# ViktorLiang/GW-Depth

Hardware: AMD Instinct MI355X
Metric: images/sec (train fwd+bwd) 480x640 bs=8/GPU (higher is better)
Workload: dtype bf16; 1 GPU; GW-Depth full model (res50 + DETR 6+6 + 4-scale ReferTransformer + decoder) fwd+17 losses+bwd+clip+AdamW, 480x640, bs=8/GPU, dropout 0.1; global_batch=8, parallelism=dp1, launch=hipgraph, graph_segments=1, grad_buckets=8

## Files before the change

### gw_depth_amd/csrc/refattn.hip

```cpp
#include "common.h"

namespace {

struct QOp {
    const void *p;
    long ws, ts, hs;
};
struct QOpW {
    void *p;
    long ws, ts, hs;
};

template <typename T, int HD>
__device__ __forceinline__ void load_row(float (&v)[HD], const T *p) {
    if constexpr (sizeof(T) == 2) {
#pragma unroll
        for (int c = 0; c < HD; c += 8) {
            const bf16x8 x = *(const bf16x8 *)(p + c);
#pragma unroll
            for (int j = 0; j < 8; ++j) v[c + j] = (float)x[j];
        }
    } else {
#pragma unroll
        for (int c = 0; c < HD; c += 4) {
            const float4 x = *(const float4 *)(p + c);
            v[c] = x.x, v[c + 1] = x.y, v[c + 2] = x.z, v[c + 3] = x.w;
        }
    }
}

template <typename T, int HD>
__global__ void ref_scores_fwd_kernel(QOp q, const T *__restrict__ refk, T *__restrict__ ra, int B, int nwin, int R, int H, float scale) {
    const long total = (long)B * nwin * 49 * H;
    const int C = H * HD, Tn = nwin * 49;
    for (long i = (long)blockIdx.x * blockDim.x + threadIdx.x; i < total; i += (long)gridDim.x * blockDim.x) {
        const int h = (int)(i % H);
        const long bt = i / H;
        const int t = (int)(bt % Tn), b = (int)(bt / Tn);
        float qv[HD];
        load_row<T, HD>(qv, (const T *)q.p + ((long)b * nwin + t / 49) * q.ws + (long)(t % 49) * q.ts + (long)h * q.hs);
        const T *kp = refk + (long)b * R * C + h * HD;
        T *dst = ra + bt * R * H + h;
        for (int r = 0; r < R; ++r) {
            float kv[HD];
            load_row<T, HD>(kv, kp + (long)r * C);
            float acc = 0.f;
#pragma unroll
            for (int d = 0; d < HD; ++d) acc += qv[d] * kv[d];
            dst[(long)r * H] = from_f32<T>(acc * scale);
        }
    }
}

template <typename T, int HD>
__global__ void ref_scores_dq_kernel(const T *__restrict__ refk, const T *__restrict__ g, QOpW dq, int B, int nwin, int R, int H, float scale) {
    const long total = (long)B * nwin * 49 * H;
    const int C = H * HD, Tn = nwin * 49;
    for (long i = (long)blockIdx.x * blockDim.x + threadIdx.x; i < total; i += (long)gridDim.x * blockDim.x) {
        const int h = (int)(i % H);
        const long bt = i / H;
        const int t = (int)(bt % Tn), b = (int)(bt / Tn);
        const T *gp = g + bt * R * H + h;
        const T *kp = refk + (long)b * R * C + h * HD;
        float acc[HD];
#pragma unroll
        for (int d = 0; d < HD; ++d) acc[d] = 0.f;
        for (int r = 0; r < R; ++r) {
            float kv[HD];
            load_row<T, HD>(kv, kp + (long)r * C);
            const float gv = to_f32(gp[(long)r * H]);
#pragma unroll
            for (int d = 0; d < HD; ++d) acc[d] += gv * kv[d];
        }
        T *dst = (T *)dq.p + ((long)b * nwin + t / 49) * dq.ws + (long)(t % 49) * dq.ts + (long)h * dq.hs;
#pragma unroll
        for (int d = 0; d < HD; ++d) dst[d] = from_f32<T>(acc[d] * scale);
    }
}

template <typename T, int HD>
__global__ void token_reduce_kernel(const T *__restrict__ a, QOp x, float *__restrict__ out, int B, int nwin, int R, int H, float scale) {
    const int lane = threadIdx.x & 63;
    const long wave = ((long)blockIdx.x * blockDim.x + threadIdx.x) >> 6, total = (long)B * R * H;
    if (wave >= total) return;
    const int h = (int)(wave % H), r = (int)((wave / H) % R), b = (int)(wave / ((long)H * R));
    const int Tn = nwin * 49;
    const T *ap = a + ((long)b * Tn * R + r) * H + h;
    float acc[HD];
#pragma unroll
    for (int d = 0; d < HD; ++d) acc[d] = 0.f;
    for (int t = lane; t < Tn; t += 64) {
        float xv[HD];
        load_row<T, HD>(xv, (const T *)x.p + ((long)b * nwin + t / 49) * x.ws + (long)(t % 49) * x.ts + (long)h * x.hs);
        const float av = to_f32(ap[(long)t * R * H]);
#pragma unroll
        for (int d = 0; d < HD; ++d) acc[d] += av * xv[d];
    }
    float *dst = out + ((long)b * R + r) * H * HD + h * HD;
#pragma unroll
    for (int d = 0; d < HD; ++d) {
        const float s = wave_sum(acc[d]);
        if (lane == (d & 63)) dst[d] = s * scale;
    }
}

template <typename T>
__global__ void ref_mix_fwd_kernel(const T *__restrict__ ra, const T *__restrict__ refv, T *__restrict__ qnew, T *__restrict__ att_out,
                                   int R, int H, int hd, int Tn) {
    extern __shared__ float sm[];
    const long bt = blockIdx.x;
    const int C = H * hd, RH = R * H;
    const T *src = ra + bt * RH;
    for (int e = threadIdx.x; e < RH; e += blockDim.x) sm[e] = to_f32(src[e]);
    __syncthreads();
    {
        float *red = sm + RH;
        const int parts = blockDim.x / H, hh = threadIdx.x % H, pp = threadIdx.x / H;
        float m = -INFINITY;
        if (pp < parts)
            for (int r = pp; r < R; r += parts) m = fmaxf(m, sm[r * H + hh]);
        if (pp < parts) red[pp * H + hh] = m;
        __syncthreads();
        for (int q = 0; q < parts; ++q) m = fmaxf(m, red[q * H + hh]);
        __syncthreads();
        float l = 0.f;
        if (pp < parts)
            for (int r = pp; r < R; r += parts) {
                const float p = __expf(sm[r * H + hh] - m);
                sm[r * H + hh] = p;
                l += p;
            }
        if (pp < parts) red[pp * H + hh] = l;
        __syncthreads();
        l = 0.f;
        for (int q = 0; q < parts; ++q) l += red[q * H + hh];
        const float inv = 1.0f / l;
        if (pp < parts)
            for (int r = pp; r < R; r += parts) sm[r * H + hh] *= inv;
    }
    __syncthreads();
    if (att_out)
        for (int e = threadIdx.x; e < RH; e += blockDim.x) att_out[bt * RH + e] = from_f32<T>(sm[e]);
    const T *vb = refv + (bt / Tn) * R * C;
    for (int e = threadIdx.x; e < C; e += blockDim.x) {
        const int h = e / hd;
        float acc = 0.f;
        for (int r = 0; r < R; ++r) acc += sm[r * H + h] * to_f32(vb[(long)r * C + e]);
        qnew[bt * C + e] = from_f32<T>(acc);
    }
}

template <typename T>
__global__ void ref_mix_bwd_kernel(const T *__restrict__ att, const T *__restrict__ refv, const T *__restrict__ g, T *__restrict__ dra,
                                   int R, int H, int hd, int Tn) {
    extern __shared__ float sm[];
    const long bt = blockIdx.x;
    const int C = H * hd, RH = R * H;
    const int GP = hd + 1;
    float *gs = sm, *da = sm + H * GP, *dot = da + RH;
    for (int e = threadIdx.x; e < C; e += blockDim.x) gs[(e / hd) * GP + e % hd] = to_f32(g[bt * C + e]);
    __syncthreads();
    const T *vb = refv + (bt / Tn) * R * C;
    constexpr int VE = 16 / (int)sizeof(T);
    const bool vec = (hd % VE) == 0 && ((uintptr_t)vb % 16) == 0;
    for (int e = threadIdx.x; e < RH; e += blockDim.x) {
        const int r = e / H, h = e % H;
        const T *vp = vb + (long)r * C + h * hd;
        float acc = 0.f;
        if (vec) {
            for (int d = 0; d < hd; d += VE) {
                const uint4 raw = *(const uint4 *)(vp + d);
                const T *pv = (const T *)&raw;
#pragma unroll
                for (int k = 0; k < VE; ++k) acc += gs[h * GP + d + k] * to_f32(pv[k]);
            }
        } else {
            for (int d = 0; d < hd; ++d) acc += gs[h * GP + d] * to_f32(vp[d]);
        }
        da[e] = acc;
    }
    __syncthreads();
    float *part = dot + H;
    const int parts = blockDim.x / H, hh = threadIdx.x % H, pp = threadIdx.x / H;
    float av[4];
    float s = 0.f;
    int n = 0;
    if (pp < parts)
        for (int r = pp; r < R; r += parts, ++n) {
            const float a = to_f32(att[bt * RH + r * H + hh]);
            if (n < 4) av[n] = a;
            s += a * da[r * H + hh];
        }
    if (pp < parts) part[pp * H + hh] = s;
    __syncthreads();
    if (threadIdx.x < H) {
        float t = 0.f;
        for (int q = 0; q < parts; ++q) t += part[q * H + threadIdx.x];
        dot[threadIdx.x] = t;
    }
    __syncthreads();
    n = 0;
    if (pp < parts)
        for (int r = pp; r < R; r += parts, ++n) {
            const float a = n < 4 ? av[n] : to_f32(att[bt * RH + r * H + hh]);
            dra[bt * RH + r * H + hh] = from_f32<T>(a * (da[r * H + hh] - dot[hh]));
        }
}

bool shape_ok(int B, int nwin, int R, int H, int hd) { return B > 0 && nwin > 0 && R > 0 && R <= 128 && H > 0 && H <= 64 && hd > 0 && hd <= 64; }
int blocks_for(long n, int per, int cap) {
    long b = (n + per - 1) / per;
    return (int)(b > cap ? cap : (b < 1 ? 1 : b));
}

}

#define HD_SWITCH(hd, CALL)            \
    switch (hd) {                      \
        case 8: { CALL(8) } break;     \
        case 16: { CALL(16) } break;   \
        case 32: { CALL(32) } break;   \
        case 64: { CALL(64) } break;   \
        default: return -4;            \
    }

bool q_aligned(const gwd_strided *q, int32_t dtype) {
    const int a = dtype == GWD_BF16 ? 8 : 4;
    return (uintptr_t)q->p % 16 == 0 && q->ws % a == 0 && q->ts % a == 0 && q->hs % a == 0;
}

extern "C" int gwd_ref_scores_forward(const gwd_strided *q, const void *ref_k, void *ra, int32_t B, int32_t nwin, int32_t R, int32_t H,
                                      int32_t hd, float scale, int32_t dtype, void *stream) {
    if (!q || !q->p || !ref_k || !ra || !shape_ok(B, nwin, R, H, hd)) return -1;
    if (!q_aligned(q, dtype) || (uintptr_t)ref_k % 16) return -5;
    const QOp qo{q->p, q->ws, q->ts, q->hs};
    const int grid = blocks_for((long)B * nwin * 49 * H, 64, 16384);
    hipStream_t s = (hipStream_t)stream;
    if (dtype == GWD_BF16) {
#define CALL(HD_) ref_scores_fwd_kernel<__bf16, HD_><<<grid, 64, 0, s>>>(qo, (const __bf16 *)ref_k, (__bf16 *)ra, B, nwin, R, H, scale);
        HD_SWITCH(hd, CALL)
#undef CALL
    } else if (dtype == GWD_F32) {
#define CALL(HD_) ref_scores_fwd_kernel<float, HD_><<<grid, 64, 0, s>>>(qo, (const float *)ref_k, (float *)ra, B, nwin, R, H, scale);
        HD_SWITCH(hd, CALL)
#undef CALL
    } else return -2;
    GWD_CHECK_LAUNCH();
    return 0;
}

extern "C" int gwd_ref_scores_backward(const gwd_strided *q, const void *ref_k, const void *g, const gwd_strided *dq, float *d_ref_k,
                                       int32_t B, int32_t nwin, int32_t R, int32_t H, int32_t hd, float scale, int32_t dtype,
                                       void *stream) {
    if (!q || !q->p || !dq || !dq->p || !ref_k || !g || !d_ref_k || !shape_ok(B, nwin, R, H, hd)) return -1;
    if (!q_aligned(q, dtype) || (uintptr_t)ref_k % 16) return -5;
    const QOp qo{q->p, q->ws, q->ts, q->hs};
    const QOpW dqo{dq->p, dq->ws, dq->ts, dq->hs};
    const int grid = blocks_for((long)B * nwin * 49 * H, 64, 16384);
    const unsigned rgrid = (unsigned)(((long)B * R * H + 3) / 4);
    hipStream_t s = (hipStream_t)stream;
    if (dtype == GWD_BF16) {
#define CALL(HD_)                                                                                                             \
    ref_scores_dq_kernel<__bf16, HD_><<<grid, 64, 0, s>>>((const __bf16 *)ref_k, (const __bf16 *)g, dqo, B, nwin, R, H, scale);    \
    token_reduce_kernel<__bf16, HD_><<<rgrid, 256, 0, s>>>((const __bf16 *)g, qo, d_ref_k, B, nwin, R, H, scale);
        HD_SWITCH(hd, CALL)
#undef CALL
    } else if (dtype == GWD_F32) {
#define CALL(HD_)                                                                                                             \
    ref_scores_dq_kernel<float, HD_><<<grid, 64, 0, s>>>((const float *)ref_k, (const float *)g, dqo, B, nwin, R, H, scale);       \
    token_reduce_kernel<float, HD_><<<rgrid, 256, 0, s>>>((const float *)g, qo, d_ref_k, B, nwin, R, H, scale);
        HD_SWITCH(hd, CALL)
#undef CALL
    } else return -2;
    GWD_CHECK_LAUNCH();
    return 0;
}

extern "C" int gwd_ref_mix_forward(const void *ra, const void *ref_v, void *q_new, void *att, int32_t B, int32_t T, int32_t R, int32_t H,
                                   int32_t hd, int32_t dtype, void *stream) {
    if (!ra || !ref_v || !q_new || T <= 0 || !shape_ok(B, 1, R, H, hd)) return -1;
    const unsigned grid = (unsigned)((long)B * T);
    hipStream_t s = (hipStream_t)stream;
    const size_t lds = ((size_t)R * H + (size_t)(256 / H) * H) * sizeof(float);
    if (dtype == GWD_BF16) ref_mix_fwd_kernel<__bf16><<<grid, 256, lds, s>>>((const __bf16 *)ra, (const __bf16 *)ref_v, (__bf16 *)q_new, (__bf16 *)att, R, H, hd, T);
    else if (dtype == GWD_F32) ref_mix_fwd_kernel<float><<<grid, 256, lds, s>>>((const float *)ra, (const float *)ref_v, (float *)q_new, (float *)att, R, H, hd, T);
    else return -2;
    GWD_CHECK_LAUNCH();
    return 0;
}

extern "C" int gwd_ref_mix_backward(const void *att, const void *ref_v, const void *g, void *d_ra, float *d_ref_v, int32_t B, int32_t T,
                                    int32_t R, int32_t H, int32_t hd, int32_t dtype, void *stream) {
    if (!att || !ref_v || !g || !d_ra || !d_ref_v || T <= 0 || T % 49 || !shape_ok(B, 1, R, H, hd)) return -1;
    if ((uintptr_t)g % 16) return -5;
    hipStream_t s = (hipStream_t)stream;
    const size_t lds = ((size_t)H * (hd + 1) + (size_t)R * H + H + (size_t)(256 / H) * H) * sizeof(float);
    const unsigned rgrid = (unsigned)(((long)B * R * H + 3) / 4);
    const long C = (long)H * hd;
    const QOp go{g, 49 * C, C, hd};
    if (dtype == GWD_BF16) {
        ref_mix_bwd_kernel<__bf16><<<(unsigned)((long)B * T), 256, lds, s>>>((const __bf16 *)att, (const __bf16 *)ref_v, (const __bf16 *)g, (__bf16 *)d_ra, R, H, hd, T);
#define CALL(HD_) token_reduce_kernel<__bf16, HD_><<<rgrid, 256, 0, s>>>((const __bf16 *)att, go, d_ref_v, B, T / 49, R, H, 1.0f);
        HD_SWITCH(hd, CALL)
#undef CALL
    } else if (dtype == GWD_F32) {
        ref_mix_bwd_kernel<float><<<(unsigned)((long)B * T), 256, lds, s>>>((const float *)att, (const float *)ref_v, (const float *)g, (float *)d_ra, R, H, hd, T);
#define CALL(HD_) token_reduce_kernel<float, HD_><<<rgrid, 256, 0, s>>>((const float *)att, go, d_ref_v, B, T / 49, R, H, 1.0f);
        HD_SWITCH(hd, CALL)
#undef CALL
    } else return -2;
    GWD_CHECK_LAUNCH();
    return 0;
}
```

Baseline: 262.2 images/s.

## Add MFMA-based token-tiled kernels for reference attention forward and backward

Adds new bf16 kernels for hd 16/32 that tile 32 tokens per block in LDS and compute the scores, the softmax-mix and their backward passes with MFMA instructions instead of scalar per-token loops. The backward launches also fold the separate token-reduction kernel into the same grid as extra blocks that do the reductions with MFMA over transposed LDS tiles. This is meant to cut launch count, scalar FMA work and redundant global reads of the reference K/V. The cost is more complex indexing, larger LDS use per block and fallback paths when alignment checks fail.

New measurement: 264.7 images/s (median of 6 runs). About the same (+1.0%).

```diff
diff --git a/gw_depth_amd/csrc/refattn.hip b/gw_depth_amd/csrc/refattn.hip
--- a/gw_depth_amd/csrc/refattn.hip
+++ b/gw_depth_amd/csrc/refattn.hip
@@ -207,6 +207,427 @@
         }
 }
 
+namespace mf {
+
+constexpr int NTHR = 512, NWV = NTHR / 64;
+constexpr int PAD = 8;
+constexpr int LDS_TOKEN_BUDGET = 61440;
+constexpr int KT = 32, PT = KT + 8;
+constexpr int SUM_COLS = 256;
+constexpr int LDS_SUM_BYTES = 2 * SUM_COLS * PT * 2;
+
+typedef __attribute__((ext_vector_type(4))) unsigned u32x4;
+typedef __attribute__((ext_vector_type(4))) __bf16 bf16x4;
+
+struct Geo {
+    int B, nwin, T, R, H;
+    int TT, ntile, P;
+    int nsum;
+};
+
+__device__ __forceinline__ f32x16 mma(const bf16x8 &a, const bf16x8 &b, const f32x16 &c) {
+    return __builtin_amdgcn_mfma_f32_32x32x16_bf16(a, b, c, 0, 0, 0);
+}
+__device__ __forceinline__ f32x16 zero16() {
+    f32x16 z;
+#pragma unroll
+    for (int i = 0; i < 16; ++i) z[i] = 0.f;
+    return z;
+}
+__device__ __forceinline__ void keep(float (&v)[8]) {
+    asm volatile("" : "+v"(v[0]), "+v"(v[1]), "+v"(v[2]), "+v"(v[3]), "+v"(v[4]), "+v"(v[5]), "+v"(v[6]), "+v"(v[7]));
+}
+__device__ __forceinline__ void keep(u32x4 (&v)[8]) {
+    asm volatile("" : "+v"(v[0]), "+v"(v[1]), "+v"(v[2]), "+v"(v[3]), "+v"(v[4]), "+v"(v[5]), "+v"(v[6]), "+v"(v[7]));
+}
+template <int KS>
+__device__ __forceinline__ void load_frags(bf16x8 (&f)[KS], const __bf16 *p, int half, bool ok) {
+    u32x4 v[KS];
+#pragma unroll
+    for (int s = 0; s < KS; ++s) v[s] = *(const u32x4 *)(p + 16 * s + 8 * half);
+    if constexpr (KS == 1) asm volatile("" : "+v"(v[0]));
+    else asm volatile("" : "+v"(v[0]), "+v"(v[1]));
+    const u32x4 z = {0u, 0u, 0u, 0u};
+#pragma unroll
+    for (int s = 0; s < KS; ++s) f[s] = __builtin_bit_cast(bf16x8, ok ? v[s] : z);
+}
+__device__ __forceinline__ int acc_row(int i, int half) { return (i & 3) + 8 * (i >> 2) + 4 * half; }
+
+__device__ __forceinline__ const __bf16 *qrow(const QOp &q, int b, int nwin, int t, int h) {
+    return (const __bf16 *)q.p + ((long)b * nwin + t / 49) * q.ws + (long)(t % 49) * q.ts + (long)h * q.hs;
+}
+
+template <bool TO_LDS>
+__device__ __forceinline__ void copy_tile(__bf16 *gl, __bf16 *img, int nrows, int rowlen, int P, bool vec) {
+    if (vec) {
+        const int ppr = rowlen >> 3, n = nrows * ppr;
+        for (int i0 = threadIdx.x; i0 < n; i0 += 4 * NTHR) {
+            u32x4 v[4], *dst[4];
+#pragma unroll
+            for (int k = 0; k < 4; ++k) {
+                const int i = min(i0 + k * NTHR, n - 1), row = i / ppr, pc = i - row * ppr;
+                u32x4 *g = (u32x4 *)(gl + (long)row * rowlen + 8 * pc), *l = (u32x4 *)(img + row * P + 8 * pc);
+                v[k] = TO_LDS ? *g : *l;
+                dst[k] = TO_LDS ? l : g;
+            }
+#pragma unroll
+            for (int k = 0; k < 4; ++k)
+                if (i0 + k * NTHR < n) *dst[k] = v[k];
+        }
+    } else {
+        const int n = nrows * rowlen;
+        for (int i = threadIdx.x; i < n; i += NTHR) {
+            const int row = i / rowlen, e = i - row * rowlen;
+            if (TO_LDS) img[row * P + e] = gl[(long)row * rowlen + e];
+            else gl[(long)row * rowlen + e] = img[row * P + e];
+        }
+    }
+}
+
+__device__ __forceinline__ void store4(__bf16 *dst, float a, float b, float c, float d) {
+    const bf16x4 o = {(__bf16)a, (__bf16)b, (__bf16)c, (__bf16)d};
+    *(bf16x4 *)dst = o;
+}
+
+template <int NW>
+__device__ __forceinline__ void load_rowv(u32x4 (&v)[NW], const __bf16 *p, bool ok) {
+#pragma unroll
+    for (int w = 0; w < NW; ++w) v[w] = *(const u32x4 *)(p + 8 * w);
+    if constexpr (NW == 2) asm volatile("" : "+v"(v[0]), "+v"(v[1]));
+    else asm volatile("" : "+v"(v[0]), "+v"(v[1]), "+v"(v[2]), "+v"(v[3]));
+    const u32x4 z = {0u, 0u, 0u, 0u};
+#pragma unroll
+    for (int w = 0; w < NW; ++w) v[w] = ok ? v[w] : z;
+}
+template <int NW>
+__device__ __forceinline__ float chan(const u32x4 (&v)[NW], int s, int half) {
+    const unsigned w = v[s >> 2][s & 3];
+    return __builtin_bit_cast(float, half ? (w & 0xffff0000u) : (w << 16));
+}
+
+template <int HD>
+__global__ __launch_bounds__(NTHR) void ref_scores_fwd_mf_kernel(QOp q, const __bf16 *__restrict__ refk, __bf16 *__restrict__ ra, Geo g,
+                                                                  float scale, bool vec) {
+    extern __shared__ __attribute__((aligned(16))) __bf16 img[];
+    constexpr int NW = HD / 8;
+    const int b = blockIdx.x / g.ntile, t0 = (blockIdx.x % g.ntile) * g.TT;
+    const int nv = min(g.TT, g.T - t0), C = g.H * HD;
+    const int lane = threadIdx.x & 63, wave = threadIdx.x >> 6, lt = lane & 31, half = lane >> 5;
+    const bool tok_ok = lt < nv;
+    const int t = t0 + (tok_ok ? lt : 0);
+    for (int h = wave; h < g.H; h += NWV) {
+        const __bf16 *qp = qrow(q, b, g.nwin, t, h);
+        u32x4 qv[NW], kv[NW];
+        load_rowv<NW>(qv, qp, tok_ok);
+        for (int r0 = 0; r0 < g.R; r0 += 32) {
+            const bool r_ok = r0 + lt < g.R;
+            const __bf16 *kp = refk + ((long)b * g.R + (r_ok ? r0 + lt : 0)) * C + h * HD;
+            f32x16 acc = zero16();
+            load_rowv<NW>(kv, kp, r_ok);
+#pragma unroll
+            for (int s = 0; s < HD / 2; ++s) acc = __builtin_amdgcn_mfma_f32_32x32x2f32(chan<NW>(kv, s, half), chan<NW>(qv, s, half), acc, 0, 0, 0);
+#pragma unroll
+            for (int i = 0; i < 16; ++i) {
+                const int r = r0 + acc_row(i, half);
+                if (r < g.R && tok_ok) img[lt * g.P + r * g.H + h] = (__bf16)(acc[i] * scale);
+            }
+        }
+    }
+    __syncthreads();
+    copy_tile<false>(ra + ((long)b * g.T + t0) * g.R * g.H, img, nv, g.R * g.H, g.P, vec);
+}
+
+template <int HD>
+__device__ __forceinline__ void token_sums(const __bf16 *__restrict__ a, const QOp &x, float *__restrict__ out, const Geo &g, int blk,
+                                           float scale, bool veca, __bf16 *smem) {
+    __bf16 *aT = smem, *xT = smem + SUM_COLS * PT;
+    const int ngrp = (g.H + 7) / 8, nrt = (g.R + 31) / 32;
+    const int rt = blk % nrt, hg = (blk / nrt) % ngrp, b = blk / (nrt * ngrp);
+    const int lane = threadIdx.x & 63, wave = threadIdx.x >> 6, lt = lane & 31, half = lane >> 5;
+    const int C = g.H * HD, RH = g.R * g.H;
+    constexpr int DB = HD / 8, XITEMS = 4 * 8 * DB;
+    const int sub = threadIdx.x >> 8, loc = threadIdx.x & 255;
+    const bool a_item = veca && loc < 128;
+    const bool x_item = loc >= 128 && loc < 128 + XITEMS;
+    const int rl = loc & 31, r_it = rt * 32 + rl, it = loc - 128, db = it % DB, hh = (it / DB) & 7, h_it = hg * 8 + hh;
+    const int tg = a_item ? loc >> 5 : it / (8 * DB);
+    const bool src_ok = a_item ? r_it < g.R : (x_item && h_it < g.H);
+    const int rc_it = min(r_it, g.R - 1), hc_it = min(h_it, g.H - 1), dbc = x_item ? db : 0;
+    __bf16 *dst = a_item ? aT + rl * PT + 8 * tg : xT + (hh * HD + 8 * db) * PT + 8 * tg;
+    const int cstride = a_item ? 32 * PT : PT;
+    auto fetch = [&](u32x4(&v)[8], int t0) {
+#pragma unroll
+        for (int j = 0; j < 8; ++j) {
+            const int t = t0 + 8 * tg + j, tc = max(0, min(t, g.T - 1));
+            const __bf16 *src = a_item ? a + ((long)b * g.T + tc) * RH + rc_it * g.H + hg * 8 : qrow(x, b, g.nwin, tc, hc_it) + 8 * dbc;
+            v[j] = *(const u32x4 *)src;
+        }
+        keep(v);
+#pragma unroll
+        for (int j = 0; j < 8; ++j) {
+            const u32x4 z = {0u, 0u, 0u, 0u};
+            v[j] = (src_ok && t0 + 8 * tg + j < g.T) ? v[j] : z;
+        }
+    };
+    f32x16 acc = zero16();
+    u32x4 v[8], vn[8];
+    fetch(v, 32 * sub);
+    for (int t0 = 0; t0 < g.T; t0 += 2 * KT) {
+        fetch(vn, t0 + 2 * KT + 32 * sub);
+        for (int s2 = 0; s2 < 2 && t0 + KT * s2 < g.T; ++s2) {
+            __syncthreads();
+            if (sub == s2 && (a_item || x_item)) {
+#pragma unroll
+                for (int c = 0; c < 8; ++c) {
+                    u32x4 y;
+#pragma unroll
+                    for (int m = 0; m < 4; ++m) {
+                        const unsigned lo = v[2 * m][c >> 1], hi = v[2 * m + 1][c >> 1];
+                        y[m] = (c & 1) ? ((lo >> 16) | (hi & 0xffff0000u)) : ((lo & 0xffffu) | (hi << 16));
+                    }
+                    *(u32x4 *)(dst + c * cstride) = y;
+                }
+            }
+            if (!veca) {
+                for (int e = threadIdx.x; e < SUM_COLS * KT; e += NTHR) {
+                    const int col = e / KT, tl = e % KT, r = rt * 32 + (col & 31), h = hg * 8 + (col >> 5), t = t0 + KT * s2 + tl;
+                    aT[col * PT + tl] = (t < g.T && r < g.R && h < g.H) ? a[((long)b * g.T + t) * RH + r * g.H + h] : (__bf16)0.f;
+                }
+            }
+            __syncthreads();
+            const __bf16 *ap = aT + (wave * 32 + lt) * PT + 8 * half, *xp = xT + (wave * HD + (lt & (HD - 1))) * PT + 8 * half;
+#pragma unroll
+            for (int s = 0; s < KT / 16; ++s) acc = mma(*(const bf16x8 *)(ap + 16 * s), *(const bf16x8 *)(xp + 16 * s), acc);
+        }
+#pragma unroll
+        for (int j = 0; j < 8; ++j) v[j] = vn[j];
+    }
+    const int h = hg * 8 + wave;
+    if (h < g.H && lt < HD) {
+#pragma unroll
+        for (int i = 0; i < 16; ++i) {
+            const int r = rt * 32 + acc_row(i, half);
+            if (r < g.R) out[((long)b * g.R + r) * C + h * HD + lt] = acc[i] * scale;
+        }
+    }
+}
+
+template <int HD>
+__global__ __launch_bounds__(NTHR) void ref_scores_bwd_mf_kernel(QOp q, const __bf16 *__restrict__ refk, const __bf16 *__restrict__ gr, QOpW dq,
+                                                                  float *__restrict__ dk, Geo g, float scale, bool vec) {
+    extern __shared__ __attribute__((aligned(16))) __bf16 img[];
+    if ((int)blockIdx.x < g.nsum) {
+        token_sums<HD>(gr, q, dk, g, blockIdx.x, scale, vec && (g.H & 7) == 0, img);
+        return;
+    }
+    const int blk = blockIdx.x - g.nsum;
+    const int b = blk / g.ntile, t0 = (blk % g.ntile) * g.TT;
+    const int nv = min(g.TT, g.T - t0), C = g.H * HD;
+    const int lane = threadIdx.x & 63, wave = threadIdx.x >> 6, lt = lane & 31, half = lane >> 5;
+    const bool tok_ok = lt < nv;
+    const int ltc = tok_ok ? lt : 0;
+    const int t = t0 + (tok_ok ? lt : 0);
+    copy_tile<true>(const_cast<__bf16 *>(gr) + ((long)b * g.T + t0) * g.R * g.H, img, nv, g.R * g.H, g.P, vec);
+    __syncthreads();
+    for (int h = wave; h < g.H; h += NWV) {
+        f32x16 acc = zero16();
+        const __bf16 *kcol = refk + (long)b * g.R * C + h * HD + (lt & (HD - 1));
+        for (int r0 = 0; r0 < g.R; r0 += 16) {
+            bf16x8 gf, kf;
+            float gv[8], kv[8];
+#pragma unroll
+            for (int j = 0; j < 8; ++j) {
+                const int rc = min(r0 + 8 * half + j, g.R - 1);
+                gv[j] = (float)img[ltc * g.P + rc * g.H + h];
+                kv[j] = (float)kcol[(long)rc * C];
+            }
+            keep(gv);
+            keep(kv);
+#pragma unroll
+            for (int j = 0; j < 8; ++j) {
+                const bool ok = r0 + 8 * half + j < g.R;
+                gf[j] = (__bf16)((ok && tok_ok) ? gv[j] : 0.f);
+                kf[j] = (__bf16)((ok && lt < HD) ? kv[j] : 0.f);
+            }
+            acc = mma(kf, gf, acc);
+        }
+        if (tok_ok) {
+            __bf16 *dst = (__bf16 *)dq.p + ((long)b * g.nwin + t / 49) * dq.ws + (long)(t % 49) * dq.ts + (long)h * dq.hs;
+#pragma unroll
+            for (int u = 0; u < HD / 8; ++u)
+                store4(dst + 8 * u + 4 * half, acc[4 * u] * scale, acc[4 * u + 1] * scale, acc[4 * u + 2] * scale, acc[4 * u + 3] * scale);
+        }
+    }
+}
+
+template <int HD>
+__global__ __launch_bounds__(NTHR) void ref_mix_fwd_mf_kernel(const __bf16 *__restrict__ ra, const __bf16 *__restrict__ refv, __bf16 *__restrict__ qnew,
+                                                               __bf16 *__restrict__ att, Geo g, bool vec_in, bool vec_out) {
+    extern __shared__ __attribute__((aligned(16))) __bf16 img[];
+    const int b = blockIdx.x / g.ntile, t0 = (blockIdx.x % g.ntile) * g.TT;
+    const int nv = min(g.TT, g.T - t0), C = g.H * HD, RH = g.R * g.H;
+    const int lane = threadIdx.x & 63, wave = threadIdx.x >> 6, lt = lane & 31, half = lane >> 5;
+    const bool tok_ok = lt < nv;
+    const int ltc = tok_ok ? lt : 0;
+    copy_tile<true>(const_cast<__bf16 *>(ra) + ((long)b * g.T + t0) * RH, img, nv, RH, g.P, vec_in);
+    __syncthreads();
+    for (int h = wave; h < g.H; h += NWV) {
+        __bf16 *row = img + ltc * g.P + h;
+        const __bf16 *vcol = refv + (long)b * g.R * C + h * HD + (lt & (HD - 1));
+        auto xs = [&](float(&xv)[8], int r0) {
+#pragma unroll
+            for (int j = 0; j < 8; ++j) xv[j] = (float)row[min(r0 + 2 * j + half, g.R - 1) * g.H];
+            keep(xv);
+#pragma unroll
+            for (int j = 0; j < 8; ++j) xv[j] = r0 + 2 * j + half < g.R ? (tok_ok ? xv[j] : 0.f) : -INFINITY;
+        };
+        auto vs = [&](float(&vv)[8], int r0) {
+#pragma unroll
+            for (int j = 0; j < 8; ++j) vv[j] = (float)vcol[(long)min(r0 + 2 * j + half, g.R - 1) * C];
+            keep(vv);
+#pragma unroll
+            for (int j = 0; j < 8; ++j) vv[j] = (r0 + 2 * j + half < g.R && lt < HD) ? vv[j] : 0.f;
+        };
+        float v[8], vn[8], xv[8];
+        vs(v, 0);
+        float m = -INFINITY;
+        for (int r0 = 0; r0 < g.R; r0 += 16) {
+            xs(xv, r0);
+#pragma unroll
+            for (int j = 0; j < 8; ++j) m = fmaxf(m, xv[j]);
+        }
+        m = fmaxf(m, __shfl_xor(m, 32, 64));
+        const int parts = 256 / g.H, nq = min(parts, g.R);
+        float l = 0.f;
+        for (int q0 = 0; q0 < nq; q0 += 8) {
+            float part[8];
+#pragma unroll
+            for (int j = 0; j < 8; ++j) part[j] = 0.f;
+            for (int rb = q0; rb < g.R; rb += parts) {
+                float e[8];
+#pragma unroll
+                for (int j = 0; j < 8; ++j) e[j] = (float)row[min(rb + j, g.R - 1) * g.H];
+                keep(e);
+#pragma unroll
+                for (int j = 0; j < 8; ++j) {
+                    const bool ok = q0 + j < nq && rb + j < g.R;
+                    part[j] += __expf((ok ? (tok_ok ? e[j] : 0.f) : -INFINITY) - m);
+                }
+            }
+#pragma unroll
+            for (int j = 0; j < 8; ++j) l += part[j];
+        }
+        const float inv = 1.0f / l;
+        f32x16 acc = zero16();
+        for (int r0 = 0; r0 < g.R; r0 += 16) {
+            vs(vn, r0 + 16);
+            xs(xv, r0);
+#pragma unroll
+            for (int j = 0; j < 8; ++j) {
+                const int r = r0 + 2 * j + half;
+                const float p = __expf(xv[j] - m) * inv;
+                if (att && tok_ok && r < g.R) row[r * g.H] = (__bf16)p;
+                if (r0 + 2 * j < g.R) acc = __builtin_amdgcn_mfma_f32_32x32x2f32(v[j], p, acc, 0, 0, 0);
+            }
+#pragma unroll
+            for (int j = 0; j < 8; ++j) v[j] = vn[j];
+        }
+        if (tok_ok) {
+            __bf16 *dst = qnew + ((long)b * g.T + t0 + lt) * C + h * HD;
+#pragma unroll
+            for (int u = 0; u < HD / 8; ++u) store4(dst + 8 * u + 4 * half, acc[4 * u], acc[4 * u + 1], acc[4 * u + 2], acc[4 * u + 3]);
+        }
+    }
+    if (att) {
+        __syncthreads();
+        copy_tile<false>(att + ((long)b * g.T + t0) * RH, img, nv, RH, g.P, vec_out);
+    }
+}
+
+template <int HD>
+__global__ __launch_bounds__(NTHR) void ref_mix_bwd_mf_kernel(const __bf16 *__restrict__ att, const __bf16 *__restrict__ refv, QOp go,
+                                                               __bf16 *__restrict__ dra, float *__restrict__ dv, Geo g, bool vec_in, bool vec_out) {
+    extern __shared__ __attribute__((aligned(16))) __bf16 img[];
+    if ((int)blockIdx.x < g.nsum) {
+        token_sums<HD>(att, go, dv, g, blockIdx.x, 1.0f, vec_in && (g.H & 7) == 0, img);
+        return;
+    }
+    constexpr int KS = HD / 16;
+    const int blk = blockIdx.x - g.nsum;
+    const int b = blk / g.ntile, t0 = (blk % g.ntile) * g.TT;
+    const int nv = min(g.TT, g.T - t0), C = g.H * HD, RH = g.R * g.H;
+    const int lane = threadIdx.x & 63, wave = threadIdx.x >> 6, lt = lane & 31, half = lane >> 5;
+    const bool tok_ok = lt < nv;
+    const int ltc = tok_ok ? lt : 0;
+    const int t = t0 + (tok_ok ? lt : 0);
+    copy_tile<true>(const_cast<__bf16 *>(att) + ((long)b * g.T + t0) * RH, img, nv, RH, g.P, vec_in);
+    __syncthreads();
+    for (int h = wave; h < g.H; h += NWV) {
+        const __bf16 *gp = qrow(go, b, g.nwin, t, h);
+        __bf16 *row = img + ltc * g.P + h;
+        bf16x8 gf[KS], vf[KS];
+        load_frags<KS>(gf, gp, half, tok_ok);
+        float dot = 0.f;
+        for (int r0 = 0; r0 < g.R; r0 += 32) {
+            const bool r_ok = r0 + lt < g.R;
+            const __bf16 *vp = refv + ((long)b * g.R + (r_ok ? r0 + lt : 0)) * C + h * HD;
+            f32x16 acc = zero16();
+            load_frags<KS>(vf, vp, half, r_ok);
+#pragma unroll
+            for (int s = 0; s < KS; ++s) acc = mma(vf[s], gf[s], acc);
+#pragma unroll
+            for (int i0 = 0; i0 < 16; i0 += 8) {
+                float av[8];
+#pragma unroll
+                for (int i = 0; i < 8; ++i) av[i] = (float)row[min(r0 + acc_row(i0 + i, half), g.R - 1) * g.H];
+                keep(av);
+#pragma unroll
+                for (int i = 0; i < 8; ++i) dot += (r0 + acc_row(i0 + i, half) < g.R && tok_ok) ? av[i] * acc[i0 + i] : 0.f;
+            }
+        }
+        dot += __shfl_xor(dot, 32, 64);
+        for (int r0 = 0; r0 < g.R; r0 += 32) {
+            const bool r_ok = r0 + lt < g.R;
+            const __bf16 *vp = refv + ((long)b * g.R + (r_ok ? r0 + lt : 0)) * C + h * HD;
+            f32x16 acc = zero16();
+            load_frags<KS>(vf, vp, half, r_ok);
+#pragma unroll
+            for (int s = 0; s < KS; ++s) acc = mma(vf[s], gf[s], acc);
+#pragma unroll
+            for (int i0 = 0; i0 < 16; i0 += 8) {
+                float av[8];
+#pragma unroll
+                for (int i = 0; i < 8; ++i) av[i] = (float)row[min(r0 + acc_row(i0 + i, half), g.R - 1) * g.H];
+                keep(av);
+#pragma unroll
+                for (int i = 0; i < 8; ++i) {
+                    const int r = r0 + acc_row(i0 + i, half);
+                    if (r < g.R && tok_ok) row[r * g.H] = (__bf16)(av[i] * (acc[i0 + i] - dot));
+                }
+            }
+        }
+    }
+    __syncthreads();
+    copy_tile<false>(dra + ((long)b * g.T + t0) * RH, img, nv, RH, g.P, vec_out);
+}
+
+bool covers(int hd, int32_t dtype) { return dtype == GWD_BF16 && (hd == 16 || hd == 32); }
+Geo geo(int B, int nwin, int T, int R, int H, bool sums) {
+    Geo g{B, nwin, T, R, H, 0, 0, R * H + PAD, 0};
+    const int tt = LDS_TOKEN_BUDGET / (g.P * 2);
+    g.TT = tt > 32 ? 32 : tt;
+    g.ntile = (T + g.TT - 1) / g.TT;
+    if (sums) g.nsum = B * ((H + 7) / 8) * ((R + 31) / 32);
+    return g;
+}
+size_t lds_bytes(const Geo &g) {
+    const size_t tok = (size_t)g.TT * g.P * 2;
+    return g.nsum && tok < (size_t)LDS_SUM_BYTES ? (size_t)LDS_SUM_BYTES : tok;
+}
+bool vec_rows(const void *p, int R, int H) { return (uintptr_t)p % 16 == 0 && (R * H) % 8 == 0; }
+
+}
+
 bool shape_ok(int B, int nwin, int R, int H, int hd) { return B > 0 && nwin > 0 && R > 0 && R <= 128 && H > 0 && H <= 64 && hd > 0 && hd <= 64; }
 int blocks_for(long n, int per, int cap) {
     long b = (n + per - 1) / per;
@@ -236,7 +657,13 @@
     const QOp qo{q->p, q->ws, q->ts, q->hs};
     const int grid = blocks_for((long)B * nwin * 49 * H, 64, 16384);
     hipStream_t s = (hipStream_t)stream;
-    if (dtype == GWD_BF16) {
+    if (mf::covers(hd, dtype)) {
+        const mf::Geo g = mf::geo(B, nwin, nwin * 49, R, H, false);
+        const unsigned mgrid = (unsigned)(B * g.ntile);
+        const bool vec = mf::vec_rows(ra, R, H);
+        if (hd == 16) mf::ref_scores_fwd_mf_kernel<16><<<mgrid, mf::NTHR, mf::lds_bytes(g), s>>>(qo, (const __bf16 *)ref_k, (__bf16 *)ra, g, scale, vec);
+        else mf::ref_scores_fwd_mf_kernel<32><<<mgrid, mf::NTHR, mf::lds_bytes(g), s>>>(qo, (const __bf16 *)ref_k, (__bf16 *)ra, g, scale, vec);
+    } else if (dtype == GWD_BF16) {
 #define CALL(HD_) ref_scores_fwd_kernel<__bf16, HD_><<<grid, 64, 0, s>>>(qo, (const __bf16 *)ref_k, (__bf16 *)ra, B, nwin, R, H, scale);
         HD_SWITCH(hd, CALL)
 #undef CALL
@@ -259,7 +686,14 @@
     const int grid = blocks_for((long)B * nwin * 49 * H, 64, 16384);
     const unsigned rgrid = (unsigned)(((long)B * R * H + 3) / 4);
     hipStream_t s = (hipStream_t)stream;
-    if (dtype == GWD_BF16) {
+    const bool dq8 = (uintptr_t)dq->p % 8 == 0 && dq->ws % 4 == 0 && dq->ts % 4 == 0 && dq->hs % 4 == 0;
+    if (mf::covers(hd, dtype) && dq8) {
+        const mf::Geo gm = mf::geo(B, nwin, nwin * 49, R, H, true);
+        const unsigned mgrid = (unsigned)(gm.nsum + B * gm.ntile);
+        const bool vec = mf::vec_rows(g, R, H);
+        if (hd == 16) mf::ref_scores_bwd_mf_kernel<16><<<mgrid, mf::NTHR, mf::lds_bytes(gm), s>>>(qo, (const __bf16 *)ref_k, (const __bf16 *)g, dqo, d_ref_k, gm, scale, vec);
+        else mf::ref_scores_bwd_mf_kernel<32><<<mgrid, mf::NTHR, mf::lds_bytes(gm), s>>>(qo, (const __bf16 *)ref_k, (const __bf16 *)g, dqo, d_ref_k, gm, scale, vec);
+    } else if (dtype == GWD_BF16) {
 #define CALL(HD_)                                                                                                             \
     ref_scores_dq_kernel<__bf16, HD_><<<grid, 64, 0, s>>>((const __bf16 *)ref_k, (const __bf16 *)g, dqo, B, nwin, R, H, scale);    \
     token_reduce_kernel<__bf16, HD_><<<rgrid, 256, 0, s>>>((const __bf16 *)g, qo, d_ref_k, B, nwin, R, H, scale);
@@ -282,7 +716,13 @@
     const unsigned grid = (unsigned)((long)B * T);
     hipStream_t s = (hipStream_t)stream;
     const size_t lds = ((size_t)R * H + (size_t)(256 / H) * H) * sizeof(float);
-    if (dtype == GWD_BF16) ref_mix_fwd_kernel<__bf16><<<grid, 256, lds, s>>>((const __bf16 *)ra, (const __bf16 *)ref_v, (__bf16 *)q_new, (__bf16 *)att, R, H, hd, T);
+    if (mf::covers(hd, dtype) && (uintptr_t)q_new % 8 == 0) {
+        const mf::Geo g = mf::geo(B, 0, T, R, H, false);
+        const unsigned mgrid = (unsigned)(B * g.ntile);
+        const bool vi = mf::vec_rows(ra, R, H), vo = mf::vec_rows(att, R, H);
+        if (hd == 16) mf::ref_mix_fwd_mf_kernel<16><<<mgrid, mf::NTHR, mf::lds_bytes(g), s>>>((const __bf16 *)ra, (const __bf16 *)ref_v, (__bf16 *)q_new, (__bf16 *)att, g, vi, vo);
+        else mf::ref_mix_fwd_mf_kernel<32><<<mgrid, mf::NTHR, mf::lds_bytes(g), s>>>((const __bf16 *)ra, (const __bf16 *)ref_v, (__bf16 *)q_new, (__bf16 *)att, g, vi, vo);
+    } else if (dtype == GWD_BF16) ref_mix_fwd_kernel<__bf16><<<grid, 256, lds, s>>>((const __bf16 *)ra, (const __bf16 *)ref_v, (__bf16 *)q_new, (__bf16 *)att, R, H, hd, T);
     else if (dtype == GWD_F32) ref_mix_fwd_kernel<float><<<grid, 256, lds, s>>>((const float *)ra, (const float *)ref_v, (float *)q_new, (float *)att, R, H, hd, T);
     else return -2;
     GWD_CHECK_LAUNCH();
@@ -298,7 +738,13 @@
     const unsigned rgrid = (unsigned)(((long)B * R * H + 3) / 4);
     const long C = (long)H * hd;
     const QOp go{g, 49 * C, C, hd};
-    if (dtype == GWD_BF16) {
+    if (mf::covers(hd, dtype) && (uintptr_t)ref_v % 16 == 0) {
+        const mf::Geo gm = mf::geo(B, T / 49, T, R, H, true);
+        const unsigned mgrid = (unsigned)(gm.nsum + B * gm.ntile);
+        const bool vi = mf::vec_rows(att, R, H), vo = mf::vec_rows(d_ra, R, H);
+        if (hd == 16) mf::ref_mix_bwd_mf_kernel<16><<<mgrid, mf::NTHR, mf::lds_bytes(gm), s>>>((const __bf16 *)att, (const __bf16 *)ref_v, go, (__bf16 *)d_ra, d_ref_v, gm, vi, vo);
+        else mf::ref_mix_bwd_mf_kernel<32><<<mgrid, mf::NTHR, mf::lds_bytes(gm), s>>>((const __bf16 *)att, (const __bf16 *)ref_v, go, (__bf16 *)d_ra, d_ref_v, gm, vi, vo);
+    } else if (dtype == GWD_BF16) {
         ref_mix_bwd_kernel<__bf16><<<(unsigned)((long)B * T), 256, lds, s>>>((const __bf16 *)att, (const __bf16 *)ref_v, (const __bf16 *)g, (__bf16 *)d_ra, R, H, hd, T);
 #define CALL(HD_) token_reduce_kernel<__bf16, HD_><<<rgrid, 256, 0, s>>>((const __bf16 *)att, go, d_ref_v, B, T / 49, R, H, 1.0f);
         HD_SWITCH(hd, CALL)
```
